# DanielMengLiu/DeepLip

Measured on AMD Instinct MI355X. Metric: lip-clips/sec (fused A+V embed), higher is better.
Workload: dtype f16x3; 1 GPU; fused A+V embed: video [64,1,29,88,88] 3D-stem+ResNet-18 + audio [64,1,80,300] E-TDNN -> z-norm concat [64,1024] per rank per step (BASELINE configs[1] clip batch); global_batch=64, parallelism=dp1, weights=random-init (name-keyed, seed 1)

## Files before the change

deeplip_amd/csrc/capi.hip:

```cpp
#include "dlip_launch.h"

extern "C" int dlip_abi_version(void) { return DLIP_ABI_VERSION; }

extern "C" const char* dlip_error_string(int code) {
  if (code == DLIP_OK) return "ok";
  if (code == DLIP_EINVAL) return "deeplip_hip: invalid argument (shape / pointer / alignment)";
  if (code == DLIP_ERANGE) return "deeplip_hip: tensor exceeds the 2 GiB single-launch addressing window";
  if (code > 0) return hipGetErrorString(static_cast<hipError_t>(code));
  return "deeplip_hip: unknown error code";
}

int dlip_dbg_value[DLIP_DBG_COUNT] = {-1, -1, -1, -1, -1, -1, -1, -1, -1, -1, -1};

extern "C" int dlip_debug_set(int32_t key, int32_t value) {
  DLIP_CHECK_ARG(key >= 0 && key < DLIP_DBG_COUNT);
  DLIP_CHECK_ARG(!(key == DLIP_DBG_ROWS2D && value > 0));
  dlip_dbg_value[key] = value;
  return DLIP_OK;
}

namespace {
int32_t* g_status_words = nullptr;
thread_local int32_t* g_status_scope = nullptr;
inline int32_t* status_now() { return g_status_scope != nullptr ? g_status_scope : g_status_words; }
}

extern "C" int32_t* dlip_status_words(void) { return status_now(); }

namespace {
struct RangeScope {
  int32_t* slots = nullptr;
  int n = 0, cur = 0, depth = 0;
};
thread_local RangeScope g_scope;

// ... 132 lines not shown
```

deeplip_amd/csrc/conv_igemm_f16x3_dma.hip:

```cpp
#include "conv_common.h"
#include "conv_dma_common.h"
#include "conv_dispatch.h"
#include "conv_dma_hooks.h"
#include <algorithm>
#include <cstdio>
#include <map>
#include <vector>
#include <mutex>
#include <utility>

namespace {

struct StreamK {
  long long iters;
  float* slabs;
  int* counters;
  int G;
  unsigned long long* span;
  int il_tiles;
  int l2_local;
  int reduce_later;
  DLIP_LAB_STREAMK_FIELDS
};

// ... 5 lines not shown
  int ho0, wo0;
  int x0;
  int w0;
  FastDiv div_howo, div_wo;
};
struct ConvGroups {
  int n, slices, tiles;
  int useful;
  ConvGroup g[kMaxGroups];
};

struct StreamKG : StreamK {
  ConvGroups grp;
};
__device__ __forceinline__ const ConvGroup& sk_group(const StreamKG& sk, int i) { return sk.grp.g[i]; }
__device__ __forceinline__ int sk_group_slices(const StreamKG& sk) { return sk.grp.slices; }
__device__ __forceinline__ int sk_group_tiles(const StreamKG& sk) { return sk.grp.tiles; }
__device__ __forceinline__ ConvGroup sk_group(const StreamK&, int) { return ConvGroup{}; }
__device__ __forceinline__ int sk_group_slices(const StreamK&) { return 0; }
__device__ __forceinline__ int sk_group_tiles(const StreamK&) { return 0; }
template <bool GROUPED> struct StreamKOf { typedef StreamK type; };
template <> struct StreamKOf<true> { typedef StreamKG type; };

template <int BM, int BN, int WAVES_M, int WAVES_N, int EPI, int NSTAGE, int OCC, bool DUAL, int VAR = 0, bool GROUPED = false>
__global__ __launch_bounds__(64 * WAVES_M* WAVES_N, OCC) void conv_igemm_f16x3_dma_kernel(const ConvArgs a, const typename StreamKOf<GROUPED>::type sk) {
  constexpr bool OSPLIT = EPI == 1;
  static_assert(!GROUPED || (BM == 256 && BN == 128 && NSTAGE == 3 && VAR == 0 && EPI != 2), "border groups: the 256 x 128 product tile, fp32 / split rows");
  constexpr int NW = WAVES_M * WAVES_N, NT = 64 * NW;
  constexpr int RPP = NT / 8;
  static_assert(BM % RPP == 0 && BN % RPP == 0, "tile rows must be whole passes");
  static_assert(NSTAGE == 2 || NSTAGE == 3, "ring depth");
  constexpr int WM = BM / WAVES_M, WN = BN / WAVES_N;
  constexpr int FR = 16;
  constexpr int MI = WM / FR, NI = WN / FR;
  constexpr int A_PER = BM / RPP, B_PER = BN / RPP;
  constexpr int NL = A_PER + B_PER;
  constexpr int STAGE_B = (BM + BN) * ROWB;
  constexpr int LDK = 32;
  constexpr int PF = NSTAGE - 1;
  constexpr int RING = NSTAGE * STAGE_B;
  static_assert(VAR == 0 || VAR == 4096, "VAR: bit 12 only");
  constexpr bool PINGPONG = BM == 256 && BN == 128 && NW == 8 && NSTAGE == 3;
  constexpr bool BIGTAPS = (VAR & 4096) != 0;
  constexpr int AQ = A_PER, BQ = B_PER;
  extern __shared__ __attribute__((aligned(16))) float smem[];

  const int nwg = gridDim.x, bid = blockIdx.x;
  const int q8 = nwg >> 3, r8 = nwg & 7, xcd = bid & 7;
  const int g_hw = (xcd < r8 ? xcd * (q8 + 1) : r8 * (q8 + 1) + (xcd - r8) * q8) + (bid >> 3);
  const int g = sk.il_tiles > 0 ? (g_hw % sk.il_tiles) * (nwg / sk.il_tiles) + g_hw / sk.il_tiles : g_hw;
// ... 24 lines not shown

  long long it_begin = 0, it_end = 0;
  bool ranged = true;
  if constexpr (GROUPED) {
    if (sk.counters == nullptr) {
      const int tn = g / sk.grp.tiles, tr = g - tn * sk.grp.tiles;
      int gi = 0;
#pragma unroll
      for (int i = 1; i < kMaxGroups; ++i) gi += tr >= sk.grp.g[i].tile0 ? 1 : 0;
      it_begin = (long long)tn * sk.grp.slices + sk.grp.g[gi].it0 + (tr - sk.grp.g[gi].tile0) * sk.grp.g[gi].nk;
      it_end = it_begin + sk.grp.g[gi].nk;
      ranged = false;
    }
  }
  if (ranged) {
    const int P = a.n_inner == 2 ? a.tiles_n : 1;
    const int gv = P > 1 ? g / P : g, Gv = P > 1 ? sk.G / P : sk.G;
    const long long itv = P > 1 ? sk.iters / P : sk.iters;
    it_begin = (long long)gv * itv / Gv;
    it_end = (long long)(gv + 1) * itv / Gv;
  }
  dlip_span_enter(sk.span, g);
  DLIP_LAB_WG_STAMP(8, true);
  for (long long it = it_begin; it < it_end;) {
    int grp_i = 0, seg_nk = a.nk, seg_tile, seg_k0;
    if constexpr (GROUPED) {
      const int tn = (int)(it / sk.grp.slices);
      const int rem = (int)(it - (long long)tn * sk.grp.slices);
#pragma unroll
      for (int i = 1; i < kMaxGroups; ++i) grp_i += rem >= sk.grp.g[i].it0 ? 1 : 0;
      seg_nk = sk.grp.g[grp_i].nk;
      const int loc = rem - sk.grp.g[grp_i].it0;
      seg_tile = loc / seg_nk;
      seg_k0 = loc - seg_tile * seg_nk;
    } else {
      seg_tile = (int)(it / a.nk);
      seg_k0 = (int)(it - (long long)seg_tile * a.nk);
    }
    const int tile = seg_tile, k0 = seg_k0;
    const int kn = (int)((it_end - it) < (long long)(seg_nk - k0) ? (it_end - it) : (long long)(seg_nk - k0));
    const int tiles_m = (a.M + BM - 1) / BM;
    int tile_n = tile / tiles_m;
    int tile_m = tile - tile_n * tiles_m;
    if constexpr (GROUPED) {
      tile_m = tile;
      tile_n = (int)(it / sk.grp.slices);
    } else
    if (a.n_inner == 2) {
      int g_o = g;
      asm volatile("" : "+s"(g_o));
      tile_m = tile;
      tile_n = g_o - (g_o / a.tiles_n) * a.tiles_n;
    } else if (a.n_inner) {
      tile_m = tile / a.tiles_n;
      tile_n = tile - tile_m * a.tiles_n;
    }
    if (it != it_begin) __syncthreads();
    DLIP_STAMP(0);
    DLIP_LAB_WG_STAMP(7, it == it_begin);

    f32x4 acc[MI][NI];
#define DLIP_FENCE() __builtin_amdgcn_sched_barrier(0)
    int a_off[AQ];
    uint32_t a_mask[AQ];
    int a_h0[BIGTAPS ? AQ : 1], a_w0[BIGTAPS ? AQ : 1];
    uint32_t a2_off[DUAL ? AQ : 1];
    auto row_of = [&](int j) { return rbase + RPP * j; };
    {
      int hi0[AQ], wi0[AQ];
      uint32_t colbits[AQ];
      if constexpr (GROUPED) {
        const ConvGroup& gr = sk.grp.g[grp_i];
#pragma unroll
        for (int j = 0; j < AQ; ++j) {
          const int m = tile_m * BM + row_of(j);
          const int mc = m < gr.M ? m : gr.M - 1;
          const int n = dlip_div(mc, gr.div_howo);
          const int rem = mc - n * gr.HoWo;
          const int ho = dlip_div(rem, gr.div_wo);
          const int wo = rem - ho * gr.Wo;
          a_off[j] = (((n * a.H + ho * a.sh) * a.W + wo * a.sw + gr.x0) * a.ldx + csrc) * 4;
          if constexpr (DUAL)
            a2_off[j] = m < gr.M ? (uint32_t)((((n * a.H2 + (gr.ho0 + ho) * a.s2h) * a.W2 + (gr.wo0 + wo) * a.s2w) * a.ldx2 + csrc) * 4) : DLIP_OOB_OFFSET;
          a_mask[j] = m < gr.M ? 0u : ~0u;
        }
      } else {
#pragma unroll
      for (int j = 0; j < AQ; ++j) {
        const int m = tile_m * BM + row_of(j);
// ... 9 lines not shown
        colbits[j] = 0u;
        a_mask[j] = 0u;
      }
      if constexpr (BIGTAPS) {
#pragma unroll
        for (int j = 0; j < AQ; ++j) {
          a_h0[j] = tile_m * BM + row_of(j) < a.M ? hi0[j] : -(1 << 28);
          a_w0[j] = wi0[j];
        }
      } else {
        for (int sx = 0; sx < a.S; ++sx)
#pragma unroll
          for (int j = 0; j < AQ; ++j) colbits[j] |= (uint32_t)((unsigned)(wi0[j] + sx * a.dw) < (unsigned)a.W) << sx;
        for (int r = 0; r < a.R; ++r)
#pragma unroll
          for (int j = 0; j < AQ; ++j)
            a_mask[j] |= ((unsigned)(hi0[j] + r * a.dh) < (unsigned)a.H ? colbits[j] : 0u) << (r * a.S);
#pragma unroll
        for (int j = 0; j < AQ; ++j)
          a_mask[j] = tile_m * BM + row_of(j) >= a.M ? ~0u : ~a_mask[j];
      }
      }
    }
    uint32_t b_off[BQ];
#pragma unroll
    for (int j = 0; j < BQ; ++j) {
      const int n = tile_n * BN + rbase + RPP * j;
      b_off[j] = n < a.K ? (uint32_t)((n * a.rsc + csrc) * 4) : DLIP_OOB_OFFSET;
      if constexpr (GROUPED) b_off[j] += (uint32_t)sk.grp.g[grp_i].w0;
    }

    int seg_nt = ntaps, seg_S = a.S, seg_nk1 = nk1, w_dr = 0, w_sub0 = 0;
    if constexpr (GROUPED) {
      seg_nt = sk.grp.g[grp_i].ntaps;
      seg_S = sk.grp.g[grp_i].S;
      seg_nk1 = seg_nk - (DUAL ? a.nk2 : 0);
      w_dr = a.S * a.Cw * 4;
      if constexpr (DUAL) w_sub0 = sk.grp.g[grp_i].w0;
    }
    int c0 = (k0 / seg_nt) * BK, tap = k0 % seg_nt;
    if constexpr (DUAL) {
      if (k0 >= seg_nk1) { c0 = a.Cw + (k0 - seg_nk1) * BK; tap = 0; }
    }
    int s_pos = tap % seg_S, x_row = (tap / seg_S) * x_dr;
    int w_row = GROUPED ? (tap / seg_S) * w_dr : 0;
    int tap_dh = (tap / a.S) * a.dh, tap_dw = s_pos * a.dw;
    int x_tap = x_row + s_pos * x_ds + c0 * 4, w_tap = GROUPED ? w_row + (s_pos * a.Cw + c0) * 4 : (tap * a.Cw + c0) * 4;
    if constexpr (BIGTAPS) { x_tap = x_row + s_pos * x_ds + (c0 / BK) * a.cs_x; w_tap = tap * a.wt + (c0 / BK) * a.cs_w; }
    if constexpr (DUAL) {
      if (c0 >= a.Cw) { x_tap = (c0 - a.Cw) * 4; w_tap = (ntaps * a.Cw + c0 - a.Cw) * 4 - w_sub0; }
    }
    auto advance = [&]() {
      if (DUAL && c0 >= a.Cw) {
        c0 += BK;
      } else {
        ++tap;
        if (++s_pos == seg_S) { s_pos = 0; x_row += x_dr; if constexpr (BIGTAPS) tap_dh += a.dh; if constexpr (GROUPED) w_row += w_dr; }
        if (tap == seg_nt) { tap = 0; s_pos = 0; x_row = 0; c0 += BK; if constexpr (BIGTAPS) tap_dh = 0; if constexpr (GROUPED) w_row = 0; }
        if constexpr (BIGTAPS) tap_dw = s_pos * a.dw;
      }
      x_tap = x_row + s_pos * x_ds + c0 * 4;
      if constexpr (GROUPED) w_tap = w_row + (s_pos * a.Cw + c0) * 4;
      else w_tap = (tap * a.Cw + c0) * 4;
      if constexpr (BIGTAPS) { x_tap = x_row + s_pos * x_ds + (c0 / BK) * a.cs_x; w_tap = tap * a.wt + (c0 / BK) * a.cs_w; }
      if (DUAL && c0 >= a.Cw) { x_tap = (c0 - a.Cw) * 4; w_tap = (ntaps * a.Cw + c0 - a.Cw) * 4 - w_sub0; }
    };
    auto tap_ok = [&](int j) -> bool {
      if constexpr (BIGTAPS) return (unsigned)(a_h0[j] + tap_dh) < (unsigned)a.H && (unsigned)(a_w0[j] + tap_dw) < (unsigned)a.W;
      else return ((a_mask[j] >> tap) & 1u) == 0u;
    };
    auto issue_a = [&](int stage) {
      const uint32_t base = piece0 + stage * STAGE_B;
      if (DUAL && c0 >= a.Cw) {
#pragma unroll
        for (int j = 0; j < A_PER; ++j)
          dma_piece(x2r, a2_off[DUAL ? j : 0] + (uint32_t)x_tap, base + j * RPP * ROWB);
        return;
      }
#pragma unroll
      for (int j = 0; j < A_PER; ++j) {
        if constexpr (BIGTAPS) {
          dma_piece(xr, tap_ok(j) ? (uint32_t)(a_off[j] + x_tap) : DLIP_OOB_OFFSET, base + j * RPP * ROWB);
        } else {
          const uint32_t oob = (a_mask[j] << (31 - tap)) & 0x80000000u;
          dma_piece(xr, (uint32_t)(a_off[j] + x_tap) | oob, base + j * RPP * ROWB);
        }
      }
    };
    auto issue_b = [&](int stage) {
      const uint32_t base = piece0 + stage * STAGE_B + BM * ROWB;
#pragma unroll
      for (int j = 0; j < B_PER; ++j)
        dma_piece(wr, b_off[j] + (uint32_t)w_tap, base + j * RPP * ROWB);
    };

    DLIP_STAMP(1);
    issue_a(0);
    issue_b(0);
    if (PF > 1 && kn > 1) {
      advance();
      issue_a(1);
      issue_b(1);
    }

#pragma unroll
    for (int mi = 0; mi < MI; ++mi)
#pragma unroll
      for (int ni = 0; ni < NI; ++ni)
#pragma unroll
        for (int e = 0; e < 4; ++e) acc[mi][ni][e] = 0.f;
    if (tid < BN) {
      const int k = tile_n * BN + tid;
      const bool kok = k < a.K;
      float* tab = smem + RING / 4;
      tab[tid] = kok ? 1.f / a.wscale[k] : 0.f;
      tab[BN + tid] = (kok && a.bias) ? a.bias[k] : 0.f;
      tab[2 * BN + tid] = (kok && a.slope) ? a.slope[k] : 1.f;
      tab[3 * BN + tid] = (kok && a.pscale) ? a.pscale[k] : 1.f;
      tab[4 * BN + tid] = (kok && a.pshift) ? a.pshift[k] : 0.f;
    }

    if constexpr (PINGPONG) {
      static_assert(NW == 8 && NSTAGE == 3, "ping-pong: eight waves, three stages");
      const bool half_b = wave >= NW / 2;
      f16x8 fal[MI], fah[MI], fbh[NI], fbl[NI];
      auto read_all = [&](int stage) {
        const float* Aw = smem + stage * (STAGE_B / 4) + a_frag;
        const float* Bw = smem + stage * (STAGE_B / 4) + b_frag;
#pragma unroll
        for (int mi = 0; mi < MI; ++mi) fal[mi] = *reinterpret_cast<const f16x8*>(Aw + mi * 16 * LDK + klo);
#pragma unroll
        for (int ni = 0; ni < NI; ++ni) fbh[ni] = *reinterpret_cast<const f16x8*>(Bw + ni * 16 * LDK + khi);
#pragma unroll
        for (int mi = 0; mi < MI; ++mi) fah[mi] = *reinterpret_cast<const f16x8*>(Aw + mi * 16 * LDK + khi);
#pragma unroll
        for (int ni = 0; ni < NI; ++ni) fbl[ni] = *reinterpret_cast<const f16x8*>(Bw + ni * 16 * LDK + klo);
      };
      auto mfma_all = [&]() {
        __builtin_amdgcn_s_setprio(2);
#pragma unroll
        for (int mi = 0; mi < MI; ++mi) {
#pragma unroll
          for (int ni = 0; ni < NI; ++ni) {
// ... 2 lines not shown
            acc[mi][ni] = __builtin_amdgcn_mfma_f32_16x16x32_f16(fbl[ni], fah[mi], acc[mi][ni], 0, 0, 0);
          }
          DLIP_FENCE();
        }
        __builtin_amdgcn_s_setprio(0);
      };
      int st_iss = (PF > 1 && kn > 1) ? 2 % NSTAGE : 1 % NSTAGE;
      auto load_phase = [&](int s) {
        read_all(s % NSTAGE);
        DLIP_FENCE();
        if (s + 2 < kn) {
          advance();
          issue_a(st_iss); issue_b(st_iss);
          st_iss = st_iss + 1 == NSTAGE ? 0 : st_iss + 1;
        }
        DLIP_FENCE();
        asm volatile("s_waitcnt lgkmcnt(0)" ::: "memory");
        DLIP_FENCE();
      };
      auto wait_next = [&](int s) {
        if (s + 1 < kn) { if (s + 2 < kn) wait_vmcnt<NL>(); else wait_vmcnt<0>(); }
      };
      DLIP_STAMP(2);
      if (PF > 1 && kn > 1) wait_vmcnt<NL>(); else wait_vmcnt<0>();
      __builtin_amdgcn_s_barrier();
      DLIP_STAMP(3);
      if (!half_b) {
        for (int s = 0; s < kn; ++s) {
          const int kt = s;
          (void)kt;
          DLIP_SSTAMP(0);
          load_phase(s);
          DLIP_SSTAMP(1);
          __builtin_amdgcn_s_barrier();
          DLIP_SSTAMP(2);
          mfma_all();
          DLIP_SSTAMP(3);
          DLIP_SSTAMP(4);
          __builtin_amdgcn_s_barrier();
          DLIP_SSTAMP(5);
          wait_next(s);
          DLIP_SSTAMP(6);
        }
      } else {
        __builtin_amdgcn_s_barrier();
        for (int s = 0; s < kn; ++s) {
          const int kt = s;
// ... 63 lines not shown
        mfma_p(0, 0, MI); DLIP_FENCE();
        DLIP_SSTAMP(2);
        if (moreP && !early) { advance(); issue_a(st_iss); } DLIP_FENCE();
        mfma_p(1, 0, MH); DLIP_FENCE();
        if (moreP && !early) { issue_b(st_iss); st_iss = st_iss + 1 == NSTAGE ? 0 : st_iss + 1; } DLIP_FENCE();
        if (MH < MI) mfma_p(1, MH, MI);
        DLIP_FENCE();
        mfma_p(2, 0, MH); DLIP_FENCE();
        DLIP_SSTAMP(3);
        if (more1) {
          if (PF > 1 && (kt + 2) < kn) wait_vmcnt<NL>(); else wait_vmcnt<0>();
          DLIP_SSTAMP(4);
          __builtin_amdgcn_s_barrier();
          DLIP_SSTAMP(5);
          read_first(st_nxt);
        }
        DLIP_FENCE();
        if (MH < MI) mfma_p(2, MH, MI);
        DLIP_FENCE();
        DLIP_SSTAMP(6);
        st_cur = st_nxt;
      }
    }
#undef DLIP_FENCE
    DLIP_STAMP(4);

    int tid_e = tid;
    asm volatile("" : "+v"(tid_e));
    const int lane_e = tid_e & 63, lrow_e = tid_e & (FR - 1), half_e = (tid_e & 63) / FR;

    int grp_e = grp_i;
    if constexpr (GROUPED) {
      grp_e = __builtin_amdgcn_readfirstlane(grp_e);
      asm volatile("" : "+s"(grp_e));
    }
    const ConvGroup& ge = sk_group(sk, grp_e);
    const int tile_nk = GROUPED ? ge.nk : a.nk;

    bool finish = true;
    if (kn != tile_nk) {
      constexpr int SLAB = BM * BN;
      volatile int* bcast = reinterpret_cast<volatile int*>(smem);
      const long long t0 = GROUPED ? (long long)tile_n * sk_group_slices(sk) + ge.it0 + (long long)tile * ge.nk : (long long)tile * a.nk;
      const int P = (!GROUPED && a.n_inner == 2) ? a.tiles_n : 1, lane_n = P > 1 ? tile_n : 0;
      const int gv = P > 1 ? g / P : g, Gv = P > 1 ? sk.G / P : sk.G;
      const long long itv = P > 1 ? sk.iters / P : sk.iters;
      const int tile_id = GROUPED ? tile_n * sk_group_tiles(sk) + ge.tile0 + tile : P > 1 ? tile * P + lane_n : tile;
      const int gf = (int)(((t0 + 1) * Gv - 1) / itv);
      const int gl = (int)(((t0 + tile_nk) * Gv - 1) / itv);
      const int others = gl - gf;
      bool l2_local = false;
      if (sk.l2_local && sk.il_tiles == 0 && q8 > 0) {
        const int big = r8 * (q8 + 1);
        const int pf = gf * P + lane_n, pl = gl * P + lane_n;
        const int xf = pf < big ? pf / (q8 + 1) : r8 + (pf - big) / q8, xl = pl < big ? pl / (q8 + 1) : r8 + (pl - big) / q8;
        l2_local = xf == xl;
      }
      if (sk.reduce_later) {
        const __amdgpu_buffer_rsrc_t sr = dlip_make_rsrc(sk.slabs + (size_t)(2 * g) * SLAB, SLAB * 4);
#pragma unroll
        for (int mi = 0; mi < MI; ++mi)
#pragma unroll
          for (int ni = 0; ni < NI; ++ni)
            __builtin_amdgcn_raw_buffer_store_b128(__builtin_bit_cast(u32x4, acc[mi][ni]), sr, ((mi * NI + ni) * NT + tid_e) * 16, 0, 0);
        finish = false;
// ... 38 lines not shown
            const __amdgpu_buffer_rsrc_t pr = dlip_make_rsrc(sk.slabs + (size_t)(2 * (p * P + lane_n) + (pb < t0 ? 1 : 0)) * SLAB, SLAB * 4);
            f32x4 v[NI];
#pragma unroll
            for (int ni = 0; ni < NI; ++ni) {
              v[ni] = acc[mi][ni];
              if (p != gv) {
                if (l2_local) v[ni] = __builtin_bit_cast(f32x4, __builtin_amdgcn_raw_buffer_load_b128(pr, ((mi * NI + ni) * NT + tid_e) * 16, 0, 1));
                else v[ni] = __builtin_bit_cast(f32x4, __builtin_amdgcn_raw_buffer_load_b128(pr, ((mi * NI + ni) * NT + tid_e) * 16, 0, 16));
              }
            }
#pragma unroll
            for (int ni = 0; ni < NI; ++ni)
#pragma unroll
              for (int c = 0; c < 4; ++c) t[ni][c] = p == gf ? v[ni][c] : t[ni][c] + v[ni][c];
            __builtin_amdgcn_sched_barrier(0);
          }
#pragma unroll
          for (int ni = 0; ni < NI; ++ni) acc[mi][ni] = t[ni];
        }
      }
      }
    }

    if (finish) {
      typedef _Float16 h4 __attribute__((ext_vector_type(4)));
      constexpr int PITCH = BN * 4;
      constexpr int CPR = BN / 4;
      constexpr int EPASS = (BM * PITCH + RING - 1) / RING;
      constexpr int PROWS = BM / EPASS;
      static_assert(BM % EPASS == 0 && PROWS % WM == 0 && PROWS * PITCH <= RING, "epilogue bands are whole wave rows");
      static_assert((PROWS * PITCH) % (NW * 1024) == 0, "a band is a whole number of DMA pieces per wave");
      static_assert(EPI != 2 || EPASS == 1, "the pooled epilogue reduces one whole-tile image");
      constexpr int RES_PIECES = PROWS * PITCH / 1024 / NW;
      constexpr int RPQ = 1024 / PITCH;
      const u32x4 rrw = make_rsrc_words(a.res, a.res ? a.r_bytes : 0u);
      const __amdgpu_buffer_rsrc_t yr = dlip_make_rsrc(a.y, a.y_bytes);
      const int kcol0 = tile_n * BN;
      char* img = reinterpret_cast<char*>(smem);
      const f32x4* tab = reinterpret_cast<const f32x4*>(smem + RING / 4);
      const bool post = a.pscale != nullptr;
      const int rows_e = GROUPED ? ge.M : a.M;
      auto out_row = [&](int m) -> int {
        if constexpr (GROUPED) {
          const int mc = m < ge.M ? m : ge.M - 1;
          const int n = dlip_div(mc, ge.div_howo);
          const int rem = mc - n * ge.HoWo;
// ... 142 lines not shown
              if (a.wg_R > 0) {
                if (m < a.M && kfirst < a.K) {
                  const int ci = dlip_div(m, a.div_howo), rem = m - ci * a.HoWo, rr = dlip_div(rem, a.div_wo), ss = rem - rr * a.Wo;
                  if (rr < a.wg_R && ss < a.wg_S) {
                    const int RS = a.wg_R * a.wg_S, crs = (a.M / a.HoWo) * RS;
                    float* dst = a.y + (size_t)kfirst * crs + ci * RS + rr * a.wg_S + ss;
#pragma unroll
                    for (int j = 0; j < 4; ++j) dst[(size_t)j * crs] = __uint_as_float(v[j]);
                  }
                }
                continue;
              }
            }
            const uint32_t off = (m < rows_e && kfirst < a.K) ? (uint32_t)((out_row(m) * a.ldy + kcol0) * 4 + c * 16) : DLIP_OOB_OFFSET;
            __builtin_amdgcn_raw_buffer_store_b128(v, yr, (int)off, 0, 0);
          }
        }
        if (ep + 1 < EPASS) __syncthreads();
      }
      if constexpr (OSPLIT) dlip_report_range(amax, a.status);
    }
    DLIP_LAB_SEGMENT_END_STAMPS();
    it += kn;
  }
  dlip_span_exit(sk.span);
  DLIP_LAB_WG_END_STAMPS();
}

template <int BM, int BN, int WAVES_M, int WAVES_N>
__global__ __launch_bounds__(256) void slab_reduce_kernel(const ConvArgs a, const float* __restrict__ slabs, int parts) {
  constexpr int NT = 64 * WAVES_M * WAVES_N, WM = BM / WAVES_M, WN = BN / WAVES_N, FR = 16;
  constexpr int MI = WM / FR, NI = WN / FR, QUADS = MI * NI * NT;
  const int q = blockIdx.x * 256 + threadIdx.x;
  if (q >= QUADS) return;
  const int tile = blockIdx.y;
  const f32x4* src = reinterpret_cast<const f32x4*>(slabs) + (size_t)2 * tile * parts * QUADS + q;
  f32x4 t = src[0];
#pragma unroll 8
  for (int p = 1; p < parts; ++p) {
    const f32x4 v = src[(size_t)2 * p * QUADS];
#pragma unroll
    for (int c = 0; c < 4; ++c) t[c] = t[c] + v[c];
  }
  const int tid = q % NT, blk = q / NT, ni = blk % NI, mi = blk / NI;
  const int wave = tid >> 6, wm = wave / WAVES_N, wn = wave % WAVES_N, lrow = tid & (FR - 1), half = (tid & 63) / FR;
  const int tiles_m = (a.M + BM - 1) / BM;
  int tile_n = tile / tiles_m, tile_m = tile - tile_n * tiles_m;
// ... 133 lines not shown
      const long long gt = (M + BM - 1) / BM;
      tiles += gt;
      slices += gt * g.nk;
      t.useful += g.ntaps * g.HoWo;
      if (slices > 0x3FFFFFFFll) return false;
    }
  for (int i = t.n; i < kMaxGroups; ++i) {
    t.g[i] = ConvGroup{};
    t.g[i].it0 = t.g[i].tile0 = 0x7FFFFFFF;
    t.g[i].nk = t.g[i].ntaps = t.g[i].S = t.g[i].M = t.g[i].HoWo = t.g[i].Wo = 1;
  }
  t.slices = (int)slices;
  t.tiles = (int)tiles;
  return true;
}

constexpr double kGroupedMinZeroShare = 0.15;
constexpr int kGroupedMinSlices = 64;
inline bool grouped_by_rule(const ConvArgs& a, const ConvGroups& gt) {
  return (double)gt.useful <= (1.0 - kGroupedMinZeroShare) * a.R * a.S * a.HoWo && a.nk - a.nk2 >= kGroupedMinSlices;
}
long long g_grouped_launches = 0;

template <int BM, int BN, int WAVES_M, int WAVES_N, int NSTAGE, int OCC, int EPI, bool DUAL, int VAR = 0, bool GROUPED = false>
int launch_one(const ConvArgs& a, hipStream_t st, const ConvGroups* groups = nullptr) {
  if constexpr (!GROUPED && BM == 256 && BN == 128 && NSTAGE == 3 && VAR == 0 && EPI != 2) {
    const int mode = dlip_dbg_value[DLIP_DBG_GROUPED];
    if (mode != 0 && dlip_dbg_value[DLIP_DBG_NINNER] <= 0) {
      ConvGroups gt;
      if (conv_groups(a, BM, &gt) && (mode > 0 || grouped_by_rule(a, gt)))
        return launch_one<BM, BN, WAVES_M, WAVES_N, NSTAGE, OCC, EPI, DUAL, VAR, true>(a, st, &gt);
    }
  }
  ConvArgs b = a;
  const int tiles_m = (a.M + BM - 1) / BM;
  b.tiles_n = (a.K + BN - 1) / BN;
  const long long tiles = GROUPED ? (long long)groups->tiles * b.tiles_n : (long long)tiles_m * b.tiles_n;
  const double nk_mean = GROUPED ? (double)groups->slices / groups->tiles : (double)a.nk;
  if (tiles <= 0 || tiles > 0x7FFFFFFFll) return DLIP_EINVAL;
  if (EPI == 2 && a.pool_group < BM) return DLIP_EINVAL;
  constexpr size_t lds = (size_t)NSTAGE * (BM + BN) * ROWB + 5 * BN * sizeof(float);
  constexpr int threads = 64 * WAVES_M * WAVES_N;
  static_assert(lds <= 160 * 1024, "LDS ring exceeds a CU");
  auto kern = conv_igemm_f16x3_dma_kernel<BM, BN, WAVES_M, WAVES_N, EPI, NSTAGE, OCC, DUAL, VAR, GROUPED>;
  int dev = 0;
  if (hipGetDevice(&dev) != hipSuccess) return DLIP_EINVAL;
  static KernelSlots ks;
  const int sl = kernel_slots(ks, dev, kern, threads, lds);
  if (sl <= 0) return DLIP_EINVAL;

  typename StreamKOf<GROUPED>::type sk;
  sk.iters = GROUPED ? (long long)groups->slices * b.tiles_n : tiles * a.nk;
  if constexpr (GROUPED) sk.grp = *groups;
  sk.slabs = nullptr;
  sk.counters = nullptr;
  long long G = tiles;
  const int balanced = dlip_dbg_value[DLIP_DBG_STREAMK] < 0 ? 1 : dlip_dbg_value[DLIP_DBG_STREAMK];
  if (balanced && tiles <= kMaxSplitTiles) {
    const double tile_us = 2.0 * BM * BN * 32.0 * nk_mean / (kSlotFlops * (WAVES_M * WAVES_N / 4.0) * 1e-6);
    const double plain_us = (double)((tiles + sl - 1) / sl) * tile_us;
    long long Gb = sl;
    if (sk.iters < 16 * Gb) Gb = sk.iters / 16 > 0 ? sk.iters / 16 : 1;
    const long long max_parts = a.nk >= 16384 ? 4 * kMaxPartsPerTile : a.nk >= 4096 ? 2 * kMaxPartsPerTile : kMaxPartsPerTile;
    const bool reduce_ok = !GROUPED && EPI == 0 && !DUAL && a.res == nullptr && a.nk >= 256 && tiles <= 64 && dlip_dbg_value[DLIP_DBG_STREAMK] != 4;
    if (Gb > tiles * max_parts && !reduce_ok) Gb = tiles * max_parts;
    const double bal_us = (double)sk.iters / Gb / nk_mean * tile_us + kHandoffUs * (BM * BN / 16384.0);
    const bool short_full = a.nk <= 16 && tiles >= sl;
// ... 120 lines not shown
extern "C" int dlip_conv_grouped_query(const int32_t* geom, int64_t* out) {
  DLIP_CHECK_ARG(geom != nullptr && out != nullptr);
  for (int i = 0; i < 12; ++i) DLIP_CHECK_ARG(geom[i] > 0 || ((i == 8 || i == 9) && geom[i] == 0));
  ConvArgs a = {};
  const int N = geom[0];
  a.H = geom[1]; a.W = geom[2]; a.C = geom[3]; a.R = geom[4]; a.S = geom[5];
  a.sh = geom[6]; a.sw = geom[7]; a.ph = geom[8]; a.pw = geom[9]; a.dh = geom[10]; a.dw = geom[11];
  a.nk2 = geom[12];
  const int Ho = (a.H + 2 * a.ph - a.dh * (a.R - 1) - 1) / a.sh + 1, Wo = (a.W + 2 * a.pw - a.dw * (a.S - 1) - 1) / a.sw + 1;
  DLIP_CHECK_ARG(Ho > 0 && Wo > 0 && a.nk2 >= 0);
  a.Wo = Wo; a.HoWo = Ho * Wo; a.M = N * a.HoWo;
  a.cchunks = (a.C + BK - 1) / BK; a.Cw = a.cchunks * BK;
  a.nk = a.R * a.S * a.cchunks + a.nk2;
  ConvGroups gt = {};
  const bool legal = a.R * a.S <= 32 && conv_groups(a, 256, &gt);
  out[0] = legal ? 1 : 0;
  out[1] = legal && grouped_by_rule(a, gt) ? 1 : 0;
  out[2] = gt.n; out[3] = gt.slices; out[4] = gt.tiles; out[5] = gt.useful;
  out[6] = (int64_t)a.R * a.S * a.HoWo;
  out[7] = g_grouped_launches;
  return DLIP_OK;
}

extern "C" int64_t dlip_conv_workspace_bytes(void) {
  int dev = 0, cus = 0;
  if (hipGetDevice(&dev) != hipSuccess || hipDeviceGetAttribute(&cus, hipDeviceAttributeMultiprocessorCount, dev) != hipSuccess)
    return -1;
  return (int64_t)kMaxSplitTiles * 4 + (int64_t)2 * cus * 160 * 256 * 4;
}

extern "C" int dlip_conv_set_workspace(void* ptr, int64_t bytes, dlip_stream_t stream) {
  hipStream_t st = static_cast<hipStream_t>(stream);
  int dev = 0;
  if (hipGetDevice(&dev) != hipSuccess) return DLIP_EINVAL;
  std::lock_guard<std::mutex> lock(ws_mutex());
  Workspace& w = ws_table()[{dev, st}];
  if (ptr == nullptr) {
    if (w.external) w = Workspace();
    return DLIP_OK;
  }
  DLIP_CHECK_ARG((reinterpret_cast<uintptr_t>(ptr) & 15) == 0 && bytes >= (int64_t)kMaxSplitTiles * 4 + 16);
  if (!w.external && (w.slabs || w.counters)) {
    if (hipStreamSynchronize(st) != hipSuccess) return DLIP_EINVAL;
    if (w.slabs) (void)hipFree(w.slabs);
    if (w.counters) (void)hipFree(w.counters);
  }
// ... 8 lines not shown
```

include/deeplip_hip.h:

```cpp
#ifndef DEEPLIP_HIP_H
#define DEEPLIP_HIP_H

#include <stdint.h>

#ifdef __cplusplus
extern "C" {
#endif

#define DLIP_ABI_VERSION 67
#define DLIP_HOST
#define DLIP_LIFT_BCAST 2048
#define DLIP_LIFT_WORDS 4098

#define DLIP_OK 0
#define DLIP_EINVAL (-1)
#define DLIP_ERANGE (-2)

typedef void* dlip_stream_t;
typedef void* dlip_plan_t;

int dlip_abi_version(void);
const char* dlip_source_sha(void);
const char* dlip_error_string(int code);

// ... 296 lines not shown
                           float scale, dlip_stream_t stream);
int dlip_stem_im2col_f32(const float* x, float* col, int32_t B, int32_t T, int32_t H, int32_t W, dlip_stream_t stream);
int dlip_stem_wgrad_operand_f32(const float* x, float* out, int64_t ld_out, int32_t B, int32_t T, int32_t H, int32_t W,
                                dlip_stream_t stream);
int dlip_split_stem_weights_f32(const float* w, float* w_img, float* w_scale, int32_t K, dlip_stream_t stream);
int dlip_dropout_keep_f32(const float* x, const float* u, float* y, int64_t n, float p, float scale, dlip_stream_t stream);
int dlip_chomp_concat_f32(DLIP_HOST const float* const* branches, DLIP_HOST const int32_t* lengths, DLIP_HOST const int32_t* widths,
                          int32_t n_branches, float* cat, int32_t B, int32_t T, int32_t backward, dlip_stream_t stream);
int dlip_mul_mask_f32(const float* x, const float* mask, float* y, int64_t n, float scale, dlip_stream_t stream);

enum { DLIP_ST_CONV = 0, DLIP_ST_STEM = 1, DLIP_ST_PACK = 2, DLIP_ST_POOL = 3, DLIP_ST_LOW = 4, DLIP_ST_COUNT = 8 };
int dlip_set_status_words(int32_t* words);
int dlip_status_scope(int32_t* words);

int dlip_span_scope_begin(uint64_t* pairs, uint64_t* acc, int32_t n);
int dlip_span_scope_end(dlip_stream_t stream, DLIP_HOST int32_t* used);

#define DLIP_EVID_WORDS 1024
#define DLIP_EVID_LINES (DLIP_EVID_WORDS / 32)
int dlip_range_scope_begin(int32_t* slots, int32_t n);
int dlip_range_scope_end(dlip_stream_t stream);

enum { DLIP_DBG_CONV_TILE = 0, DLIP_DBG_DMA_TILE = 1, DLIP_DBG_DMA_ENABLE = 2, DLIP_DBG_STREAMK = 3, DLIP_DBG_WIN = 4, DLIP_DBG_NINNER = 5,
       DLIP_DBG_ROWS = 6, DLIP_DBG_ROWS2D = 7, DLIP_DBG_BN_FUSED = 8, DLIP_DBG_ROWS_TAIL = 9, DLIP_DBG_GROUPED = 10, DLIP_DBG_COUNT = 11 };
int dlip_debug_set(int32_t key, int32_t value);

int dlip_shuffle_stem24_f32(const float* x, const float* w_248x32, const float* bias, const float* slope, float* y,
                            int32_t B, int32_t T, int32_t H, int32_t W, dlip_stream_t stream);
int dlip_shuffle_dwpw_f32(const float* x, const float* dw_w, const float* dw_b, const float* w, const float* bias,
                          const float* xp, float* y, int32_t N, int32_t H, int32_t W, int32_t stride, int32_t Cin,
                          int32_t K, int32_t Kp, int32_t ldx, int32_t ldp, int32_t ldy, int32_t hp, int32_t par,
                          dlip_stream_t stream);
int dlip_avgpool3_nhwc_f32(const float* x, float* y, int32_t N, int32_t H, int32_t W, int32_t C, dlip_stream_t stream);

int dlip_tcn_dw_fwd_f32(const float* x, int32_t n, DLIP_HOST const float* const* w, DLIP_HOST const float* const* bias,
                        DLIP_HOST const float* const* slope, DLIP_HOST float* const* y, DLIP_HOST const int32_t* k,
                        DLIP_HOST const int32_t* pad, DLIP_HOST const int32_t* t_out, int32_t B, int32_t T, int32_t C, int32_t d,
                        dlip_stream_t stream);
int dlip_tcn_dw_dgrad_f32(DLIP_HOST const float* const* dz, int32_t n, DLIP_HOST const float* const* w, DLIP_HOST const int32_t* k,
                          DLIP_HOST const int32_t* pad, DLIP_HOST const int32_t* t_out, float* dx, int32_t B, int32_t T, int32_t C,
                          int32_t d, dlip_stream_t stream);
int dlip_tcn_dw_wgrad_chunks(int32_t rows);
int dlip_tcn_dw_wgrad_f32(const float* x, int32_t n, DLIP_HOST const float* const* dz, DLIP_HOST float* const* dw,
                          DLIP_HOST const int32_t* k, DLIP_HOST const int32_t* pad, DLIP_HOST const int32_t* t_out, int32_t B, int32_t T,
                          int32_t C, int32_t d, double* workspace, int64_t workspace_len, dlip_stream_t stream);

int dlip_triplet_mine_f32(const float* x, const int32_t* labels, float margin, int32_t mode, const float* u, float* g,
// ... 133 lines not shown
```

Baseline: 16630 lip-clips/sec.

## Add register epilogue and early next-tile prologue to ping-pong conv kernel

```diff
diff --git a/deeplip_amd/csrc/capi.hip b/deeplip_amd/csrc/capi.hip
--- a/deeplip_amd/csrc/capi.hip
+++ b/deeplip_amd/csrc/capi.hip
@@ -10,7 +10,7 @@
   return "deeplip_hip: unknown error code";
 }
 
-int dlip_dbg_value[DLIP_DBG_COUNT] = {-1, -1, -1, -1, -1, -1, -1, -1, -1, -1, -1};
+int dlip_dbg_value[DLIP_DBG_COUNT] = {-1, -1, -1, -1, -1, -1, -1, -1, -1, -1, -1, -1};
 
 extern "C" int dlip_debug_set(int32_t key, int32_t value) {
   DLIP_CHECK_ARG(key >= 0 && key < DLIP_DBG_COUNT);
diff --git a/deeplip_amd/csrc/conv_igemm_f16x3_dma.hip b/deeplip_amd/csrc/conv_igemm_f16x3_dma.hip
--- a/deeplip_amd/csrc/conv_igemm_f16x3_dma.hip
+++ b/deeplip_amd/csrc/conv_igemm_f16x3_dma.hip
@@ -51,10 +51,12 @@
 template <bool GROUPED> struct StreamKOf { typedef StreamK type; };
 template <> struct StreamKOf<true> { typedef StreamKG type; };
 
-template <int BM, int BN, int WAVES_M, int WAVES_N, int EPI, int NSTAGE, int OCC, bool DUAL, int VAR = 0, bool GROUPED = false>
+template <int BM, int BN, int WAVES_M, int WAVES_N, int EPI, int NSTAGE, int OCC, bool DUAL, int VAR = 0, bool GROUPED = false, int HEAD = 0>
 __global__ __launch_bounds__(64 * WAVES_M* WAVES_N, OCC) void conv_igemm_f16x3_dma_kernel(const ConvArgs a, const typename StreamKOf<GROUPED>::type sk) {
   constexpr bool OSPLIT = EPI == 1;
   static_assert(!GROUPED || (BM == 256 && BN == 128 && NSTAGE == 3 && VAR == 0 && EPI != 2), "border groups: the 256 x 128 product tile, fp32 / split rows");
+  static_assert(HEAD == 0 || (HEAD <= 2 && BM == 256 && BN == 128 && WAVES_M * WAVES_N == 8 && NSTAGE == 3 && VAR == 0 && EPI == 1),
+                "register epilogue / early head: the ping-pong tile, split-format rows");
   constexpr int NW = WAVES_M * WAVES_N, NT = 64 * NW;
   constexpr int RPP = NT / 8;
   static_assert(BM % RPP == 0 && BN % RPP == 0, "tile rows must be whole passes");
@@ -125,7 +127,15 @@
   }
   dlip_span_enter(sk.span, g);
   DLIP_LAB_WG_STAMP(8, true);
-  for (long long it = it_begin; it < it_end;) {
+  struct Seg { int grp, nk, tile, k0, kn, tile_m, tile_n; };
+  int a_off[AQ];
+  uint32_t a_mask[AQ];
+  int a_h0[BIGTAPS ? AQ : 1], a_w0[BIGTAPS ? AQ : 1];
+  uint32_t a2_off[DUAL ? AQ : 1];
+  uint32_t b_off[BQ];
+  int seg_nt = ntaps, seg_S = a.S, seg_nk1 = nk1, w_dr = 0, w_sub0 = 0;
+  int c0 = 0, tap = 0, s_pos = 0, x_row = 0, w_row = 0, tap_dh = 0, tap_dw = 0, x_tap = 0, w_tap = 0;
+  auto seg_decode = [&](const long long it) __attribute__((always_inline)) -> Seg {
     int grp_i = 0, seg_nk = a.nk, seg_tile, seg_k0;
     if constexpr (GROUPED) {
       const int tn = (int)(it / sk.grp.slices);
@@ -158,16 +168,83 @@
       tile_m = tile / a.tiles_n;
       tile_n = tile - tile_m * a.tiles_n;
     }
-    if (it != it_begin) __syncthreads();
-    DLIP_STAMP(0);
-    DLIP_LAB_WG_STAMP(7, it == it_begin);
-
-    f32x4 acc[MI][NI];
+    return Seg{grp_i, seg_nk, tile, k0, kn, tile_m, tile_n};
+  };
 #define DLIP_FENCE() __builtin_amdgcn_sched_barrier(0)
-    int a_off[AQ];
-    uint32_t a_mask[AQ];
-    int a_h0[BIGTAPS ? AQ : 1], a_w0[BIGTAPS ? AQ : 1];
-    uint32_t a2_off[DUAL ? AQ : 1];
+  auto advance = [&]() {
+    if (DUAL && c0 >= a.Cw) {
+      c0 += BK;
+    } else {
+      ++tap;
+      if (++s_pos == seg_S) { s_pos = 0; x_row += x_dr; if constexpr (BIGTAPS) tap_dh += a.dh; if constexpr (GROUPED) w_row += w_dr; }
+      if (tap == seg_nt) { tap = 0; s_pos = 0; x_row = 0; c0 += BK; if constexpr (BIGTAPS) tap_dh = 0; if constexpr (GROUPED) w_row = 0; }
+      if constexpr (BIGTAPS) tap_dw = s_pos * a.dw;
+    }
+    x_tap = x_row + s_pos * x_ds + c0 * 4;
+    if constexpr (GROUPED) w_tap = w_row + (s_pos * a.Cw + c0) * 4;
+    else w_tap = (tap * a.Cw + c0) * 4;
+    if constexpr (BIGTAPS) { x_tap = x_row + s_pos * x_ds + (c0 / BK) * a.cs_x; w_tap = tap * a.wt + (c0 / BK) * a.cs_w; }
+    if (DUAL && c0 >= a.Cw) { x_tap = (c0 - a.Cw) * 4; w_tap = (ntaps * a.Cw + c0 - a.Cw) * 4 - w_sub0; }
+  };
+  auto tap_ok = [&](int j) -> bool {
+    if constexpr (BIGTAPS) return (unsigned)(a_h0[j] + tap_dh) < (unsigned)a.H && (unsigned)(a_w0[j] + tap_dw) < (unsigned)a.W;
+    else return ((a_mask[j] >> tap) & 1u) == 0u;
+  };
+  auto issue_a = [&](int stage) {
+    const uint32_t base = piece0 + stage * STAGE_B;
+    if (DUAL && c0 >= a.Cw) {
+#pragma unroll
+      for (int j = 0; j < A_PER; ++j)
+        dma_piece(x2r, a2_off[DUAL ? j : 0] + (uint32_t)x_tap, base + j * RPP * ROWB);
+      return;
+    }
+#pragma unroll
+    for (int j = 0; j < A_PER; ++j) {
+      if constexpr (BIGTAPS) {
+        dma_piece(xr, tap_ok(j) ? (uint32_t)(a_off[j] + x_tap) : DLIP_OOB_OFFSET, base + j * RPP * ROWB);
+      } else {
+        const uint32_t oob = (a_mask[j] << (31 - tap)) & 0x80000000u;
+        dma_piece(xr, (uint32_t)(a_off[j] + x_tap) | oob, base + j * RPP * ROWB);
+      }
+    }
+  };
+  auto issue_b = [&](int stage) {
+    const uint32_t base = piece0 + stage * STAGE_B + BM * ROWB;
+#pragma unroll
+    for (int j = 0; j < B_PER; ++j)
+      dma_piece(wr, b_off[j] + (uint32_t)w_tap, base + j * RPP * ROWB);
+  };
+  constexpr int TAB_F = 5 * BN;
+  float tab_v[HEAD >= 1 ? 5 : 1] = {};
+  (void)tab_v;
+  auto tab_fetch = [&](const int tile_n) __attribute__((always_inline)) {
+    if constexpr (HEAD >= 1) {
+      const int k = tile_n * BN + tid;
+      if (tid < BN && k < a.K) {
+        tab_v[0] = a.wscale[k];
+        tab_v[1] = a.bias ? a.bias[k] : 0.f;
+        tab_v[2] = a.slope ? a.slope[k] : 1.f;
+        tab_v[3] = a.pscale ? a.pscale[k] : 1.f;
+        tab_v[4] = a.pshift ? a.pshift[k] : 0.f;
+      }
+    }
+  };
+  auto tab_store = [&](const int tab_i, const int tile_n) __attribute__((always_inline)) {
+    if constexpr (HEAD >= 1) {
+      if (tid < BN) {
+        const bool kok = tile_n * BN + tid < a.K;
+        float* tab = smem + RING / 4 + tab_i * TAB_F;
+        tab[tid] = kok ? 1.f / tab_v[0] : 0.f;
+        tab[BN + tid] = kok ? tab_v[1] : 0.f;
+        tab[2 * BN + tid] = kok ? tab_v[2] : 1.f;
+        tab[3 * BN + tid] = kok ? tab_v[3] : 1.f;
+        tab[4 * BN + tid] = kok ? tab_v[4] : 0.f;
+      }
+    }
+  };
+  auto seg_fill = [&](const Seg& sg, const bool first) __attribute__((always_inline)) {
+    const int grp_i = sg.grp, seg_nk = sg.nk, k0 = sg.k0, kn = sg.kn, tile_m = sg.tile_m, tile_n = sg.tile_n;
+    tab_fetch(tile_n);
     auto row_of = [&](int j) { return rbase + RPP * j; };
     {
       int hi0[AQ], wi0[AQ];
@@ -223,7 +300,6 @@
       }
       }
     }
-    uint32_t b_off[BQ];
 #pragma unroll
     for (int j = 0; j < BQ; ++j) {
       const int n = tile_n * BN + rbase + RPP * j;
@@ -231,7 +307,7 @@
       if constexpr (GROUPED) b_off[j] += (uint32_t)sk.grp.g[grp_i].w0;
     }
 
-    int seg_nt = ntaps, seg_S = a.S, seg_nk1 = nk1, w_dr = 0, w_sub0 = 0;
+    seg_nt = ntaps; seg_S = a.S; seg_nk1 = nk1; w_dr = 0; w_sub0 = 0;
     if constexpr (GROUPED) {
       seg_nt = sk.grp.g[grp_i].ntaps;
       seg_S = sk.grp.g[grp_i].S;
@@ -239,63 +315,24 @@
       w_dr = a.S * a.Cw * 4;
       if constexpr (DUAL) w_sub0 = sk.grp.g[grp_i].w0;
     }
-    int c0 = (k0 / seg_nt) * BK, tap = k0 % seg_nt;
+    c0 = (k0 / seg_nt) * BK; tap = k0 % seg_nt;
     if constexpr (DUAL) {
       if (k0 >= seg_nk1) { c0 = a.Cw + (k0 - seg_nk1) * BK; tap = 0; }
     }
-    int s_pos = tap % seg_S, x_row = (tap / seg_S) * x_dr;
-    int w_row = GROUPED ? (tap / seg_S) * w_dr : 0;
-    int tap_dh = (tap / a.S) * a.dh, tap_dw = s_pos * a.dw;
-    int x_tap = x_row + s_pos * x_ds + c0 * 4, w_tap = GROUPED ? w_row + (s_pos * a.Cw + c0) * 4 : (tap * a.Cw + c0) * 4;
+    s_pos = tap % seg_S; x_row = (tap / seg_S) * x_dr;
+    w_row = GROUPED ? (tap / seg_S) * w_dr : 0;
+    tap_dh = (tap / a.S) * a.dh; tap_dw = s_pos * a.dw;
+    x_tap = x_row + s_pos * x_ds + c0 * 4; w_tap = GROUPED ? w_row + (s_pos * a.Cw + c0) * 4 : (tap * a.Cw + c0) * 4;
     if constexpr (BIGTAPS) { x_tap = x_row + s_pos * x_ds + (c0 / BK) * a.cs_x; w_tap = tap * a.wt + (c0 / BK) * a.cs_w; }
     if constexpr (DUAL) {
       if (c0 >= a.Cw) { x_tap = (c0 - a.Cw) * 4; w_tap = (ntaps * a.Cw + c0 - a.Cw) * 4 - w_sub0; }
     }
-    auto advance = [&]() {
-      if (DUAL && c0 >= a.Cw) {
-        c0 += BK;
-      } else {
-        ++tap;
-        if (++s_pos == seg_S) { s_pos = 0; x_row += x_dr; if constexpr (BIGTAPS) tap_dh += a.dh; if constexpr (GROUPED) w_row += w_dr; }
-        if (tap == seg_nt) { tap = 0; s_pos = 0; x_row = 0; c0 += BK; if constexpr (BIGTAPS) tap_dh = 0; if constexpr (GROUPED) w_row = 0; }
-        if constexpr (BIGTAPS) tap_dw = s_pos * a.dw;
-      }
-      x_tap = x_row + s_pos * x_ds + c0 * 4;
-      if constexpr (GROUPED) w_tap = w_row + (s_pos * a.Cw + c0) * 4;
-      else w_tap = (tap * a.Cw + c0) * 4;
-      if constexpr (BIGTAPS) { x_tap = x_row + s_pos * x_ds + (c0 / BK) * a.cs_x; w_tap = tap * a.wt + (c0 / BK) * a.cs_w; }
-      if (DUAL && c0 >= a.Cw) { x_tap = (c0 - a.Cw) * 4; w_tap = (ntaps * a.Cw + c0 - a.Cw) * 4 - w_sub0; }
-    };
-    auto tap_ok = [&](int j) -> bool {
-      if constexpr (BIGTAPS) return (unsigned)(a_h0[j] + tap_dh) < (unsigned)a.H && (unsigned)(a_w0[j] + tap_dw) < (unsigned)a.W;
-      else return ((a_mask[j] >> tap) & 1u) == 0u;
-    };
-    auto issue_a = [&](int stage) {
-      const uint32_t base = piece0 + stage * STAGE_B;
-      if (DUAL && c0 >= a.Cw) {
-#pragma unroll
-        for (int j = 0; j < A_PER; ++j)
-          dma_piece(x2r, a2_off[DUAL ? j : 0] + (uint32_t)x_tap, base + j * RPP * ROWB);
-        return;
-      }
-#pragma unroll
-      for (int j = 0; j < A_PER; ++j) {
-        if constexpr (BIGTAPS) {
-          dma_piece(xr, tap_ok(j) ? (uint32_t)(a_off[j] + x_tap) : DLIP_OOB_OFFSET, base + j * RPP * ROWB);
-        } else {
-          const uint32_t oob = (a_mask[j] << (31 - tap)) & 0x80000000u;
-          dma_piece(xr, (uint32_t)(a_off[j] + x_tap) | oob, base + j * RPP * ROWB);
-        }
-      }
-    };
-    auto issue_b = [&](int stage) {
-      const uint32_t base = piece0 + stage * STAGE_B + BM * ROWB;
-#pragma unroll
-      for (int j = 0; j < B_PER; ++j)
-        dma_piece(wr, b_off[j] + (uint32_t)w_tap, base + j * RPP * ROWB);
-    };
-
-    DLIP_STAMP(1);
+
+    {
+      const long long it = first ? it_begin : it_begin - 1;
+      (void)it;
+      DLIP_STAMP(1);
+    }
     issue_a(0);
     issue_b(0);
     if (PF > 1 && kn > 1) {
@@ -303,13 +340,7 @@
       issue_a(1);
       issue_b(1);
     }
-
-#pragma unroll
-    for (int mi = 0; mi < MI; ++mi)
-#pragma unroll
-      for (int ni = 0; ni < NI; ++ni)
-#pragma unroll
-        for (int e = 0; e < 4; ++e) acc[mi][ni][e] = 0.f;
+    if constexpr (HEAD == 0)
     if (tid < BN) {
       const int k = tile_n * BN + tid;
       const bool kok = k < a.K;
@@ -320,6 +351,28 @@
       tab[3 * BN + tid] = (kok && a.pscale) ? a.pscale[k] : 1.f;
       tab[4 * BN + tid] = (kok && a.pshift) ? a.pshift[k] : 0.f;
     }
+  };
+
+  Seg seg_cur = {};
+  bool headed = false;
+  int tab_cur = 0;
+  for (long long it = it_begin; it < it_end;) {
+    if (HEAD < 2 || !headed) {
+      seg_cur = seg_decode(it);
+      if (it != it_begin) __syncthreads();
+      DLIP_STAMP(0);
+      DLIP_LAB_WG_STAMP(7, it == it_begin);
+      seg_fill(seg_cur, it == it_begin);
+    }
+    const int grp_i = seg_cur.grp, tile = seg_cur.tile, kn = seg_cur.kn, tile_m = seg_cur.tile_m, tile_n = seg_cur.tile_n;
+
+    f32x4 acc[MI][NI];
+#pragma unroll
+    for (int mi = 0; mi < MI; ++mi)
+#pragma unroll
+      for (int ni = 0; ni < NI; ++ni)
+#pragma unroll
+        for (int e = 0; e < 4; ++e) acc[mi][ni][e] = 0.f;
 
     if constexpr (PINGPONG) {
       static_assert(NW == 8 && NSTAGE == 3, "ping-pong: eight waves, three stages");
@@ -368,7 +421,8 @@
         if (s + 1 < kn) { if (s + 2 < kn) wait_vmcnt<NL>(); else wait_vmcnt<0>(); }
       };
       DLIP_STAMP(2);
-      if (PF > 1 && kn > 1) wait_vmcnt<NL>(); else wait_vmcnt<0>();
+      if (PF > 1 && kn > 1 && !(HEAD == 2 && headed)) wait_vmcnt<NL>(); else wait_vmcnt<0>();
+      tab_store(tab_cur, tile_n);
       __builtin_amdgcn_s_barrier();
       DLIP_STAMP(3);
       if (!half_b) {
@@ -478,8 +532,13 @@
         st_cur = st_nxt;
       }
     }
-#undef DLIP_FENCE
     DLIP_STAMP(4);
+
+    const bool head_next = HEAD == 2 && it + kn < it_end;
+    if (head_next) {
+      seg_cur = seg_decode(it + kn);
+      seg_fill(seg_cur, false);
+    }
 
     int tid_e = tid;
     asm volatile("" : "+v"(tid_e));
@@ -496,7 +555,7 @@
     bool finish = true;
     if (kn != tile_nk) {
       constexpr int SLAB = BM * BN;
-      volatile int* bcast = reinterpret_cast<volatile int*>(smem);
+      volatile int* bcast = reinterpret_cast<volatile int*>(smem + (HEAD == 2 ? RING / 4 + 2 * TAB_F : 0));
       const long long t0 = GROUPED ? (long long)tile_n * sk_group_slices(sk) + ge.it0 + (long long)tile * ge.nk : (long long)tile * a.nk;
       const int P = (!GROUPED && a.n_inner == 2) ? a.tiles_n : 1, lane_n = P > 1 ? tile_n : 0;
       const int gv = P > 1 ? g / P : g, Gv = P > 1 ? sk.G / P : sk.G;
@@ -581,6 +640,90 @@
       }
     }
 
+    if constexpr (HEAD >= 1) {
+      if (finish) {
+        typedef _Float16 h8 __attribute__((ext_vector_type(8)));
+        static_assert(OSPLIT && PINGPONG && NI % 2 == 0, "register epilogue: split-format rows of the ping-pong tile");
+        const f32x4* tab = reinterpret_cast<const f32x4*>(smem + RING / 4 + tab_cur * TAB_F);
+        const __amdgpu_buffer_rsrc_t rr = dlip_make_rsrc(a.res, a.res ? a.r_bytes : 0u);
+        const __amdgpu_buffer_rsrc_t yr = dlip_make_rsrc(a.y, a.y_bytes);
+        const bool post = a.pscale != nullptr;
+        const int kcol0 = tile_n * BN;
+        const int rows_e = GROUPED ? ge.M : a.M;
+        const int cs = ((half_e & 1) << 4) | ((half_e & 2) << 2);
+        int orow[MI];
+#pragma unroll
+        for (int mi = 0; mi < MI; ++mi) {
+          const int m = tile_m * BM + wm * WM + mi * FR + lrow_e;
+          int r = m;
+          if constexpr (GROUPED) {
+            const int mc = m < ge.M ? m : ge.M - 1;
+            const int n = dlip_div(mc, ge.div_howo);
+            const int rem = mc - n * ge.HoWo;
+            const int ho = dlip_div(rem, ge.div_wo);
+            r = n * a.HoWo + (ge.ho0 + ho) * a.Wo + ge.wo0 + (rem - ho * ge.Wo);
+          }
+          orow[mi] = m < rows_e ? r : -1;
+        }
+        h8 rh[MI] = {}, rl[MI] = {};
+        auto res_fetch = [&](int p, int mi) {
+          const int kb = kcol0 + wn * WN + 32 * p;
+          const bool ok = orow[mi] >= 0 && kb < a.K;
+          const uint32_t off = ok ? (uint32_t)((orow[mi] * a.ldr + kb) * 4 + cs * 2) : DLIP_OOB_OFFSET;
+          rh[mi] = __builtin_bit_cast(h8, __builtin_amdgcn_raw_buffer_load_b128(rr, (int)off, 0, 0));
+          rl[mi] = __builtin_bit_cast(h8, __builtin_amdgcn_raw_buffer_load_b128(rr, (int)(ok ? off + 64u : DLIP_OOB_OFFSET), 0, 0));
+        };
+        if (a.res) {
+#pragma unroll
+          for (int mi = 0; mi < MI; ++mi) res_fetch(0, mi);
+        }
+        float amax = 0.f;
+#pragma unroll
+        for (int p = 0; p < NI / 2; ++p) {
+          const int kl = wn * WN + 32 * p + cs;
+          float inv[8], bi[8], sl[8], ps[8], pt[8];
+#pragma unroll
+          for (int q = 0; q < 2; ++q) {
+            const f32x4 i4 = tab[(kl >> 2) + q], b4 = tab[((BN + kl) >> 2) + q], l4 = tab[((2 * BN + kl) >> 2) + q];
+            f32x4 p4 = {1.f, 1.f, 1.f, 1.f}, t4 = {0.f, 0.f, 0.f, 0.f};
+            if (post) { p4 = tab[((3 * BN + kl) >> 2) + q]; t4 = tab[((4 * BN + kl) >> 2) + q]; }
+#pragma unroll
+            for (int c = 0; c < 4; ++c) { inv[4 * q + c] = i4[c]; bi[4 * q + c] = b4[c]; sl[4 * q + c] = l4[c]; ps[4 * q + c] = p4[c]; pt[4 * q + c] = t4[c]; }
+          }
+#pragma unroll
+          for (int mi = 0; mi < MI; ++mi) {
+            float v[8];
+#pragma unroll
+            for (int c = 0; c < 4; ++c) {
+              const float xc = acc[mi][2 * p][c], yc = acc[mi][2 * p + 1][c];
+              const auto r = __builtin_amdgcn_permlane16_swap(__float_as_uint(xc), __float_as_uint(yc), false, false);
+              v[c] = __uint_as_float(r[0]);
+              v[4 + c] = __uint_as_float(r[1]);
+            }
+            const h8 rhv = rh[mi], rlv = rl[mi];
+            if (a.res && p + 1 < NI / 2) res_fetch(p + 1, mi);
+            h8 hi, lo;
+#pragma unroll
+            for (int c = 0; c < 8; ++c) {
+              float t = v[c] * inv[c] + bi[c];
+              if (a.res) t += (float)rhv[c] + (float)rlv[c];
+              t = t >= 0.f ? t : t * sl[c];
+              if (post) t = t * ps[c] + pt[c];
+              hi[c] = (_Float16)t;
+              lo[c] = (_Float16)(t - (float)hi[c]);
+              amax = fmaxf(amax, fabsf(t));
+            }
+            const int kb = kcol0 + wn * WN + 32 * p;
+            const bool ok = orow[mi] >= 0 && kb < a.K;
+            const uint32_t off = ok ? (uint32_t)((orow[mi] * a.ldy + kb) * 4 + cs * 2) : DLIP_OOB_OFFSET;
+            __builtin_amdgcn_raw_buffer_store_b128(__builtin_bit_cast(u32x4, hi), yr, (int)off, 0, 0);
+            __builtin_amdgcn_raw_buffer_store_b128(__builtin_bit_cast(u32x4, lo), yr, (int)(ok ? off + 64u : DLIP_OOB_OFFSET), 0, 0);
+          }
+          __builtin_amdgcn_sched_barrier(0);
+        }
+        dlip_report_range(amax, a.status);
+      }
+    } else
     if (finish) {
       typedef _Float16 h4 __attribute__((ext_vector_type(4)));
       constexpr int PITCH = BN * 4;
@@ -769,7 +912,10 @@
     }
     DLIP_LAB_SEGMENT_END_STAMPS();
     it += kn;
-  }
+    headed = head_next;
+    if (head_next) tab_cur ^= 1;
+  }
+#undef DLIP_FENCE
   dlip_span_exit(sk.span);
   DLIP_LAB_WG_END_STAMPS();
 }
@@ -949,7 +1095,14 @@
 }
 long long g_grouped_launches = 0;
 
-template <int BM, int BN, int WAVES_M, int WAVES_N, int NSTAGE, int OCC, int EPI, bool DUAL, int VAR = 0, bool GROUPED = false>
+constexpr int kRingHeadBuiltIn = 1;
+inline int ring_head_route() {
+  const int v = dlip_dbg_value[DLIP_DBG_RING_HEAD];
+  return v >= 0 && v <= 2 ? v : kRingHeadBuiltIn;
+}
+long long g_ring_head_launches[3] = {};
+
+template <int BM, int BN, int WAVES_M, int WAVES_N, int NSTAGE, int OCC, int EPI, bool DUAL, int VAR = 0, bool GROUPED = false, int HEAD = 0>
 int launch_one(const ConvArgs& a, hipStream_t st, const ConvGroups* groups = nullptr) {
   if constexpr (!GROUPED && BM == 256 && BN == 128 && NSTAGE == 3 && VAR == 0 && EPI != 2) {
     const int mode = dlip_dbg_value[DLIP_DBG_GROUPED];
@@ -959,6 +1112,12 @@
         return launch_one<BM, BN, WAVES_M, WAVES_N, NSTAGE, OCC, EPI, DUAL, VAR, true>(a, st, &gt);
     }
   }
+  if constexpr (HEAD == 0 && BM == 256 && BN == 128 && WAVES_M * WAVES_N == 8 && NSTAGE == 3 && VAR == 0 && EPI == 1) {
+    const int route = ring_head_route();
+    if (route == 1) return launch_one<BM, BN, WAVES_M, WAVES_N, NSTAGE, OCC, EPI, DUAL, VAR, GROUPED, 1>(a, st, groups);
+    if (route == 2) return launch_one<BM, BN, WAVES_M, WAVES_N, NSTAGE, OCC, EPI, DUAL, VAR, GROUPED, 2>(a, st, groups);
+  }
+  if constexpr (BM == 256 && BN == 128 && WAVES_M * WAVES_N == 8 && NSTAGE == 3 && VAR == 0 && EPI == 1) ++g_ring_head_launches[HEAD];
   ConvArgs b = a;
   const int tiles_m = (a.M + BM - 1) / BM;
   b.tiles_n = (a.K + BN - 1) / BN;
@@ -966,10 +1125,10 @@
   const double nk_mean = GROUPED ? (double)groups->slices / groups->tiles : (double)a.nk;
   if (tiles <= 0 || tiles > 0x7FFFFFFFll) return DLIP_EINVAL;
   if (EPI == 2 && a.pool_group < BM) return DLIP_EINVAL;
-  constexpr size_t lds = (size_t)NSTAGE * (BM + BN) * ROWB + 5 * BN * sizeof(float);
+  constexpr size_t lds = (size_t)NSTAGE * (BM + BN) * ROWB + 5 * BN * sizeof(float) + (HEAD == 2 ? 5 * BN * sizeof(float) + 16 : 0);
   constexpr int threads = 64 * WAVES_M * WAVES_N;
   static_assert(lds <= 160 * 1024, "LDS ring exceeds a CU");
-  auto kern = conv_igemm_f16x3_dma_kernel<BM, BN, WAVES_M, WAVES_N, EPI, NSTAGE, OCC, DUAL, VAR, GROUPED>;
+  auto kern = conv_igemm_f16x3_dma_kernel<BM, BN, WAVES_M, WAVES_N, EPI, NSTAGE, OCC, DUAL, VAR, GROUPED, HEAD>;
   int dev = 0;
   if (hipGetDevice(&dev) != hipSuccess) return DLIP_EINVAL;
   static KernelSlots ks;
@@ -1136,6 +1295,13 @@
   return DLIP_OK;
 }
 
+extern "C" int dlip_conv_ring_head_query(int64_t* out) {
+  DLIP_CHECK_ARG(out != nullptr);
+  for (int i = 0; i < 3; ++i) out[i] = g_ring_head_launches[i];
+  out[3] = kRingHeadBuiltIn;
+  return DLIP_OK;
+}
+
 extern "C" int64_t dlip_conv_workspace_bytes(void) {
   int dev = 0, cus = 0;
   if (hipGetDevice(&dev) != hipSuccess || hipDeviceGetAttribute(&cus, hipDeviceAttributeMultiprocessorCount, dev) != hipSuccess)
diff --git a/include/deeplip_hip.h b/include/deeplip_hip.h
--- a/include/deeplip_hip.h
+++ b/include/deeplip_hip.h
@@ -342,7 +342,8 @@
 int dlip_range_scope_end(dlip_stream_t stream);
 
 enum { DLIP_DBG_CONV_TILE = 0, DLIP_DBG_DMA_TILE = 1, DLIP_DBG_DMA_ENABLE = 2, DLIP_DBG_STREAMK = 3, DLIP_DBG_WIN = 4, DLIP_DBG_NINNER = 5,
-       DLIP_DBG_ROWS = 6, DLIP_DBG_ROWS2D = 7, DLIP_DBG_BN_FUSED = 8, DLIP_DBG_ROWS_TAIL = 9, DLIP_DBG_GROUPED = 10, DLIP_DBG_COUNT = 11 };
+       DLIP_DBG_ROWS = 6, DLIP_DBG_ROWS2D = 7, DLIP_DBG_BN_FUSED = 8, DLIP_DBG_ROWS_TAIL = 9, DLIP_DBG_GROUPED = 10, DLIP_DBG_RING_HEAD = 11,
+       DLIP_DBG_COUNT = 12 };
 int dlip_debug_set(int32_t key, int32_t value);
 
 int dlip_shuffle_stem24_f32(const float* x, const float* w_248x32, const float* bias, const float* slope, float* y,
```

New measurement: 16990 lip-clips/sec (median of 6 runs). 2.2% higher.
